# lucidrains/vector-quantize-pytorch

Measured on NVIDIA H100. Metric: vectors quantized/sec at dim=256, codebook=1024; indices bit-exact vs ref, higher is better.
Workload: dtype bf16

## Files before the change

### vector_quantize_pytorch_b200/csrc/epilogue.cuh

```cuda
#pragma once
#include <stdint.h>

namespace vqb {

__host__ __device__ __forceinline__ int group_col(int e) { return ((e >> 1) << 3) | (e & 1); }

__device__ __forceinline__ float fmax3(float a, float b, float c) { return fmaxf(fmaxf(a, b), c); }
template <int G>
__device__ __forceinline__ float max_group(const uint32_t* r) {
  static_assert(G == 4 || G == 8 || G == 16, "group size");
  if (G == 4) return fmaxf(fmax3(__uint_as_float(r[0]), __uint_as_float(r[1]), __uint_as_float(r[2])), __uint_as_float(r[3]));
  if (G == 8)
    return fmax3(fmax3(__uint_as_float(r[0]), __uint_as_float(r[1]), __uint_as_float(r[2])),
                 fmax3(__uint_as_float(r[3]), __uint_as_float(r[4]), __uint_as_float(r[5])),
                 fmaxf(__uint_as_float(r[6]), __uint_as_float(r[7])));
  const float a = fmax3(__uint_as_float(r[0]), __uint_as_float(r[1]), __uint_as_float(r[2]));
  const float b = fmax3(__uint_as_float(r[3]), __uint_as_float(r[4]), __uint_as_float(r[5]));
  const float c = fmax3(__uint_as_float(r[6]), __uint_as_float(r[7]), __uint_as_float(r[8]));
  const float d = fmax3(__uint_as_float(r[9]), __uint_as_float(r[10]), __uint_as_float(r[11]));
  const float e = fmax3(__uint_as_float(r[12]), __uint_as_float(r[13]), __uint_as_float(r[14]));
  return fmaxf(fmax3(a, b, c), fmax3(d, e, __uint_as_float(r[15])));
}
__device__ __forceinline__ float max16(const uint32_t (&r)[16]) { return max_group<16>(r); }

// ... 9 lines not shown
  template <int G>
  __device__ __forceinline__ void insert(const uint32_t* r, int cbase, uint32_t tagmask, uint32_t mul1, uint32_t mulm1) {
    const float o1 = t1, o2 = t2, o3 = t3;
#pragma unroll
    for (int e = 0; e < G; ++e) {
      const uint32_t ku = (r[e] & tagmask) | static_cast<uint32_t>(15 - e);
      const float n1 = fmaxf(t1, __uint_as_float(ku));
      const uint32_t lo1 = __float_as_uint(n1) * mulm1 + (__float_as_uint(t1) * mul1 + ku);
      const float n2 = fmaxf(t2, __uint_as_float(lo1));
      const uint32_t lo2 = __float_as_uint(n2) * mulm1 + (__float_as_uint(t2) * mul1 + lo1);
      const float n3 = fmaxf(t3, __uint_as_float(lo2));
      const uint32_t lo3 = __float_as_uint(n3) * mulm1 + (__float_as_uint(t3) * mul1 + lo2);
      t4 = fmaxf(t4, __uint_as_float(lo3));
      t1 = n1;
      t2 = n2;
      t3 = n3;
    }
    const int k1 = j1, k2 = j2, k3 = j3;
    const bool m1 = t1 == o1;
    j1 = m1 ? k1 : cbase;
    const float q2 = m1 ? o2 : o1;
    const bool m2 = t2 == q2;
    j2 = m2 ? (m1 ? k2 : k1) : cbase;
    const int used = static_cast<int>(m1) + static_cast<int>(m2);
    const float q3 = used == 0 ? o1 : (used == 1 ? o2 : o3);
    j3 = (t3 == q3) ? (used == 0 ? k1 : (used == 1 ? k2 : k3)) : cbase;
    thr = t1 - W;
  }
  __device__ __forceinline__ void piece(const uint32_t (&r)[16], int cbase, uint32_t tagmask, uint32_t mul1, uint32_t mulm1) {
    insert<16>(r, cbase, tagmask, mul1, mulm1);
  }
  static __device__ __forceinline__ int col(float t, int j) { return j + group_col(15 - static_cast<int>(__float_as_uint(t) & 15u)); }
};

struct MergeSlot { float t1, t2, t3, t4, bexact; int i0, i1, i2; };

struct RowResult { int i0, i1, i2, n; float best; };

struct Top3 {
  float v0 = -3.4e38f, v1 = -3.4e38f, v2 = -3.4e38f;
  int i0 = 0, i1 = 0, i2 = 0;
  __device__ __forceinline__ void offer(float v, int i) {
    if (v > v0 || (v == v0 && i < i0)) { v2 = v1; i2 = i1; v1 = v0; i1 = i0; v0 = v; i0 = i; }
    else if (v > v1 || (v == v1 && i < i1)) { v2 = v1; i2 = i1; v1 = v; i1 = i; }
    else if (v > v2 || (v == v2 && i < i2)) { v2 = v; i2 = i; }
  }
};

__device__ __forceinline__ void publish(MergeSlot* slot, const RowState& st) {
  slot->t1 = st.t1; slot->t2 = st.t2; slot->t3 = st.t3; slot->t4 = st.t4; slot->bexact = st.bexact;
  slot->i0 = RowState::col(st.t1, st.j1); slot->i1 = RowState::col(st.t2, st.j2); slot->i2 = RowState::col(st.t3, st.j3);
}

__device__ __forceinline__ RowResult merge_slices(const RowState& st, const MergeSlot* slots, int nslots, int stride) {
  float best = st.bexact, tb = st.t1;
  int ib = RowState::col(st.t1, st.j1);
  for (int q = 0; q < nslots; ++q) {
    const MergeSlot& m = slots[q * stride];
    best = fmaxf(best, m.bexact);
    const bool take = m.t1 > tb || (m.t1 == tb && m.i0 < ib);
    tb = take ? m.t1 : tb;
    ib = take ? m.i0 : ib;
  }
  const float band = tb - st.W;
  int n = (st.t1 > band) + (st.t2 > band) + (st.t3 > band) + (st.t4 > band);
  for (int q = 0; q < nslots; ++q) {
    const MergeSlot& m = slots[q * stride];
    n += (m.t1 > band) + (m.t2 > band) + (m.t3 > band) + (m.t4 > band);
  }
  RowResult r;
  r.i0 = ib; r.i1 = 0; r.i2 = 0; r.n = n; r.best = best;
  if (n >= 2) {
    Top3 top;
    top.offer(st.t1, RowState::col(st.t1, st.j1));
    top.offer(st.t2, RowState::col(st.t2, st.j2));
    top.offer(st.t3, RowState::col(st.t3, st.j3));
    for (int q = 0; q < nslots; ++q) {
      const MergeSlot& m = slots[q * stride];
      top.offer(m.t1, m.i0);
      top.offer(m.t2, m.i1);
      top.offer(m.t3, m.i2);
    }
    r.i0 = top.i0; r.i1 = top.i1; r.i2 = top.i2;
  }
  return r;
}

template <int G>
struct ScanQueue {
  static constexpr int CAP = 4;
  uint4 v[CAP + 1][G / 4];
  int c[CAP + 1];
};

template <int G>
struct ScanState {
  static constexpr int CAP = ScanQueue<G>::CAP;
  float t1;
  float thr;
  float kill;
  float W;
  int cnt;

  __device__ __forceinline__ void init(float w) {
    W = w; t1 = -3.4e38f; thr = -3.4e38f; kill = -3.4e38f; cnt = 0;
  }
  __device__ __forceinline__ void raise(float other) { thr = fmaxf(thr, other - W); }

  __device__ __forceinline__ void push(ScanQueue<G>& q, const uint32_t* r, int col, float m, bool p) {
    const int c0 = (m > kill) ? 0 : cnt;
    const int slot = min(c0, CAP);
    if (p) {
#pragma unroll
      for (int e = 0; e < G; e += 4) q.v[slot][e >> 2] = make_uint4(r[e], r[e + 1], r[e + 2], r[e + 3]);
      q.c[slot] = col;
    }
    cnt = p ? min(c0 + 1, CAP + 1) : cnt;
    t1 = fmaxf(t1, m);
    thr = fmaxf(thr, t1 - W);
    kill = t1 + W;
  }

  template <bool BRANCH = true>
  __device__ __forceinline__ void scan16(ScanQueue<G>& q, const uint32_t (&r)[16], int cbase) {
    float m[16 / G];
    bool any = false;
#pragma unroll
    for (int g = 0; g < 16 / G; ++g) {
      m[g] = max_group<G>(r + g * G);
// ... 112 lines not shown
```

### vector_quantize_pytorch_b200/csrc/ptx.cuh

```cuda
#pragma once
#include <cuda.h>
#include <cuda_runtime.h>
#include <stdint.h>

namespace vqb {

__device__ __forceinline__ uint32_t smem_u32(const void* p) {
  return static_cast<uint32_t>(__cvta_generic_to_shared(p));
}

__device__ __forceinline__ void mbar_init(uint32_t bar, uint32_t count) {
  asm volatile("mbarrier.init.shared::cta.b64 [%0], %1;" ::"r"(bar), "r"(count));
}
__device__ __forceinline__ void fence_barrier_init() {
  asm volatile("fence.mbarrier_init.release.cluster;" ::: "memory");
}
__device__ __forceinline__ void mbar_arrive(uint32_t bar) {
  asm volatile("mbarrier.arrive.shared::cta.b64 _, [%0];" ::"r"(bar) : "memory");
}
__device__ __forceinline__ void mbar_arrive_expect_tx(uint32_t bar, uint32_t bytes) {
  asm volatile("mbarrier.arrive.expect_tx.shared::cta.b64 _, [%0], %1;" ::"r"(bar), "r"(bytes) : "memory");
}
__device__ __forceinline__ bool mbar_try_wait(uint32_t bar, uint32_t parity) {
  uint32_t ok;
  asm volatile(
      "{\n"
      ".reg .pred p;\n"
      "mbarrier.try_wait.parity.shared::cta.b64 p, [%1], %2;\n"
      "selp.u32 %0, 1, 0, p;\n"
      "}\n"
      : "=r"(ok)
      : "r"(bar), "r"(parity)
      : "memory");
  return ok != 0;
}

#ifndef VQB_WAIT_TIMEOUT_CYCLES
#define VQB_WAIT_TIMEOUT_CYCLES (8000000000ll)
#endif
__device__ __forceinline__ void mbar_wait(uint32_t bar, uint32_t parity) {
  if (mbar_try_wait(bar, parity)) return;
  const long long t0 = clock64();
  while (!mbar_try_wait(bar, parity)) {
    if (clock64() - t0 > VQB_WAIT_TIMEOUT_CYCLES) __trap();
  }
}

__device__ __forceinline__ void tma_prefetch_desc(const CUtensorMap* m) {
  asm volatile("prefetch.tensormap [%0];" ::"l"(reinterpret_cast<uint64_t>(m)) : "memory");
}
__device__ __forceinline__ void tma_load_3d(uint32_t dst, const CUtensorMap* m, uint32_t bar, int c0, int c1, int c2) {
  asm volatile(
      "cp.async.bulk.tensor.3d.shared::cluster.global.tile.mbarrier::complete_tx::bytes [%0], [%1, {%3, %4, %5}], [%2];"
      ::"r"(dst), "l"(reinterpret_cast<uint64_t>(m)), "r"(bar), "r"(c0), "r"(c1), "r"(c2)
      : "memory");
}

__device__ __forceinline__ void tma_prefetch_l2_3d(const CUtensorMap* m, int c0, int c1, int c2) {
  asm volatile("cp.async.bulk.prefetch.tensor.3d.L2.global.tile [%0, {%1, %2, %3}];"
               ::"l"(reinterpret_cast<uint64_t>(m)), "r"(c0), "r"(c1), "r"(c2)
               : "memory");
}

__device__ __forceinline__ uint64_t wgmma_desc_sw128(uint32_t saddr) {
  uint64_t d = 0;
  d |= static_cast<uint64_t>((saddr >> 4) & 0x3FFF);
  d |= static_cast<uint64_t>(1) << 16;
  d |= static_cast<uint64_t>(1024 >> 4) << 32;
  d |= static_cast<uint64_t>(1) << 62;
  return d;
}

__device__ __forceinline__ uint64_t wgmma_desc_sw32(uint32_t saddr) {
  uint64_t d = 0;
  d |= static_cast<uint64_t>((saddr >> 4) & 0x3FFF);
  d |= static_cast<uint64_t>(1) << 16;
  d |= static_cast<uint64_t>(256 >> 4) << 32;
  d |= static_cast<uint64_t>(3) << 62;
  return d;
}

__device__ __forceinline__ void fence_proxy_async_shared() { asm volatile("fence.proxy.async.shared::cta;" ::: "memory"); }
__device__ __forceinline__ void wgmma_fence() { asm volatile("wgmma.fence.sync.aligned;" ::: "memory"); }
__device__ __forceinline__ void wgmma_commit() { asm volatile("wgmma.commit_group.sync.aligned;" ::: "memory"); }
template <int N>
__device__ __forceinline__ void wgmma_wait() { asm volatile("wgmma.wait_group.sync.aligned %0;" ::"n"(N) : "memory"); }

template <int R>
__device__ __forceinline__ void fence_regs(float (&d)[R]) {
#pragma unroll
  for (int i = 0; i < R; ++i) asm volatile("" : "+f"(d[i])::"memory");
}

__device__ __forceinline__ void wgmma_m64n128k16_bf16(float (&d)[64], uint64_t adesc, uint64_t bdesc) {
  asm volatile(
      "{\n"
      "wgmma.mma_async.sync.aligned.m64n128k16.f32.bf16.bf16 "
      "{%0, %1, %2, %3, %4, %5, %6, %7, %8, %9, %10, %11, %12, %13, %14, %15, "
// ... 147 lines not shown
```

### vector_quantize_pytorch_b200/csrc/vq_assign.cu

```cuda
#include <type_traits>
#include "ptx.cuh"
#include "vqb_common.cuh"
#include "gather_row.cuh"
#include "epilogue.cuh"

#ifdef VQB_PROFILE
#define PROF_CLOCK() clock64()
#else
#define PROF_CLOCK() 0ll
#endif

namespace vqb {

constexpr int BM = 128;
constexpr int WM = 64;
constexpr int BN_STAGE = 128;
constexpr int BK = 64;
constexpr int A_SUB_BYTES = BM * BK * 2;
constexpr int B_SUB_BYTES = BN_STAGE * BK * 2;
constexpr int MAX_A_SUB = 8;
constexpr int MAX_STAGES = 8;
constexpr int NUM_CONSUMER_WARPS = 8;
constexpr int NUM_STORE_WARPS = 3;
constexpr int NUM_THREADS = 128 + NUM_CONSUMER_WARPS * 32;
constexpr int SMEM_CTRL_BYTES = 14336;
constexpr int SMEM_LIMIT = 232448;
constexpr int SEED_BYTES = BN_STAGE * 32;

struct AssignParams {
  int64_t N;
  int D, K, Kpad;
  int n_a, n_passes;
  int KB;
  int n_stages;
  int n_seed;
  int stream_a;
  const uint16_t* a_global;
  const uint16_t* bext;
  int num_row_tiles, num_code_steps;
  float margin_rel;
  const float* cmax;
  int32_t* idx;
  int32_t* idx_prov;
  int32_t* hist;
  int hist_shift;
  vqb_flag_entry* flagged;
  int32_t* flag_count;
  float* dbg_best;
  const uint8_t* row_mask;
  long long* prof;
  FusedOut fo;
  int copy_mode;
  int resid_mode;
  int metric;
  const uint16_t* b_hi;
  const float* cnorm2;
  uint32_t tagmask, mul1, mulm1;
};

struct Ctrl {
  uint64_t a_full[MAX_A_SUB], a_empty[MAX_A_SUB];
  uint64_t b_full[MAX_STAGES], b_empty[MAX_STAGES];
  uint64_t g_full[2], g_empty[2];
  int gidx[2][BM];
  MergeSlot merge[BM][3];
  float x2[BM];
};
static_assert(sizeof(Ctrl) <= SMEM_CTRL_BYTES, "control block too large");

template <int GB>
__device__ __forceinline__ float tail_rows(const FusedOut& fo, const int64_t (&rows)[GB], const int (&ks)[GB], int D, int lane) {
  if (fo.dtype == VQB_DTYPE_BF16) return gather_rows<VQB_DTYPE_BF16, GB>(fo, rows, ks, D, lane);
  return gather_rows<VQB_DTYPE_F32, GB>(fo, rows, ks, D, lane);
}

__device__ __forceinline__ float sq_diff16(const uint4& xa, const uint4& ca, bool bf) {
  const uint32_t xw[4] = {xa.x, xa.y, xa.z, xa.w}, cw[4] = {ca.x, ca.y, ca.z, ca.w};
  float s = 0.f;
#pragma unroll
  for (int e = 0; e < 4; ++e) {
    if (bf) {
      const float d0 = __uint_as_float(xw[e] << 16) - __uint_as_float(cw[e] << 16);
      const float d1 = __uint_as_float(xw[e] & 0xFFFF0000u) - __uint_as_float(cw[e] & 0xFFFF0000u);
      s += bf16_round(d0 * d0);
      s += bf16_round(d1 * d1);
    } else {
      const float d = __uint_as_float(xw[e]) - __uint_as_float(cw[e]);
      s += d * d;
    }
  }
  return s;
}

template <int WN>
struct StepLocals {
  float loss_ = 0.f;
  __device__ __forceinline__ float& loss() { return loss_; }
};
template <>
struct StepLocals<256> {
  static __device__ __forceinline__ float& loss() {
    __shared__ float s[NUM_CONSUMER_WARPS * 32];
    return s[threadIdx.x - 128];
  }
  static __device__ __forceinline__ uint32_t* bias_ones() {
    __shared__ __align__(256) uint32_t o[WM * 16 / 2];
    return o;
  }
  __device__ __forceinline__ StepLocals() { loss() = 0.f; }
};
constexpr int WIDE_STATIC_SMEM = NUM_CONSUMER_WARPS * 32 * 4 + WM * 16 * 2;

template <int TAIL, int WN>
__global__ void __launch_bounds__(NUM_THREADS, 1)
vq_assign_kernel(const __grid_constant__ CUtensorMap tmA, const __grid_constant__ CUtensorMap tmB,
                 const __grid_constant__ CUtensorMap tmS, const AssignParams p) {
  static_assert(WN == 128 || WN == 256, "code step width");
  constexpr int SPAN = WN / BN_STAGE;
  constexpr uint32_t STEP_SEED_BYTES = SPAN * SEED_BYTES;
  extern __shared__ __align__(1024) uint8_t smem[];
  Ctrl* ctrl = reinterpret_cast<Ctrl*>(smem);
  const uint32_t smem_base = smem_u32(smem);
  const uint32_t a_base = (smem_base + SMEM_CTRL_BYTES + 1023u) & ~1023u;
  const bool stream_a = WN == 128 && p.stream_a;
  const int n_sub = stream_a ? 0 : p.n_a * p.KB;
  const uint32_t b_base = a_base + n_sub * A_SUB_BYTES;
  const uint32_t a_stage_bytes = stream_a ? A_SUB_BYTES : 0;
  const uint32_t stage_stride = a_stage_bytes + SPAN * B_SUB_BYTES;
  const int n_ring = p.n_stages / SPAN;
  const uint32_t seed_base = b_base + n_ring * stage_stride;

  const int warp = threadIdx.x >> 5;
  const int lane = threadIdx.x & 31;

  if (threadIdx.x == 0) {
    tma_prefetch_desc(&tmA);
    tma_prefetch_desc(&tmB);
    tma_prefetch_desc(&tmS);
    for (int s = 0; s < n_sub; ++s) {
      mbar_init(smem_u32(&ctrl->a_full[s]), 1);
      mbar_init(smem_u32(&ctrl->a_empty[s]), NUM_CONSUMER_WARPS);
    }
    for (int s = 0; s < n_ring; ++s) {
      mbar_init(smem_u32(&ctrl->b_full[s]), 1);
      mbar_init(smem_u32(&ctrl->b_empty[s]), NUM_CONSUMER_WARPS);
    }
    for (int s = 0; s < 2; ++s) {
      mbar_init(smem_u32(&ctrl->g_full[s]), NUM_CONSUMER_WARPS);
      mbar_init(smem_u32(&ctrl->g_empty[s]), NUM_STORE_WARPS);
    }
    fence_barrier_init();
  }
  if constexpr (WN == 256) {
    for (int i = threadIdx.x; i < WM * 16 / 2; i += NUM_THREADS) StepLocals<256>::bias_ones()[i] = 0x3F803F80u;
    fence_proxy_async_shared();
  }
  __syncthreads();

  if (warp == 0) {
    if (lane == 0) {
      long long w_empty = 0, w_aempty = 0;
      const long long pstart = PROF_CLOCK();
      int stage = 0, gstep = 0;
      uint32_t ph = 0;
      for (int t = 0, tile = static_cast<int>(blockIdx.x); tile < p.num_row_tiles; ++t, tile += static_cast<int>(gridDim.x)) {
        const int row0 = tile * BM;
        if (!stream_a && tile + static_cast<int>(gridDim.x) < p.num_row_tiles) {
          for (int ap = 0; ap < p.n_a; ++ap)
            for (int kb = 0; kb < p.KB; ++kb) tma_prefetch_l2_3d(&tmA, kb * BK, row0 + static_cast<int>(gridDim.x) * BM, ap);
        }
        for (int ct = 0; ct < p.num_code_steps; ++ct, ++gstep) {
          for (int kb = 0; kb < p.KB; ++kb) {
            for (int ps = 0; ps < p.n_passes; ++ps) {
              const int bplane = (ps == 1) ? 1 : 0;
              const int aplane = (ps == 2) ? 1 : 0;
              if (!stream_a && ct == 0 && (ps == 0 || ps == 2)) {
                const int sub = aplane * p.KB + kb;
                { const long long c0 = PROF_CLOCK(); mbar_wait(smem_u32(&ctrl->a_empty[sub]), (t & 1) ^ 1); w_aempty += PROF_CLOCK() - c0; }
                mbar_arrive_expect_tx(smem_u32(&ctrl->a_full[sub]), A_SUB_BYTES);
                tma_load_3d(a_base + sub * A_SUB_BYTES, &tmA, smem_u32(&ctrl->a_full[sub]), kb * BK, row0, aplane);
              }
              { const long long c0 = PROF_CLOCK(); mbar_wait(smem_u32(&ctrl->b_empty[stage]), ph ^ 1); w_empty += PROF_CLOCK() - c0; }
              const bool seeds = kb == 0 && ps == 0;
              mbar_arrive_expect_tx(smem_u32(&ctrl->b_full[stage]), stage_stride + (seeds ? STEP_SEED_BYTES : 0));
              if (seeds)
                tma_load_3d(seed_base + (gstep % p.n_seed) * STEP_SEED_BYTES, &tmS, smem_u32(&ctrl->b_full[stage]), 0, ct * WN, 0);
              if (stream_a)
                tma_load_3d(b_base + stage * stage_stride, &tmA, smem_u32(&ctrl->b_full[stage]), kb * BK, row0, aplane);
              tma_load_3d(b_base + stage * stage_stride + a_stage_bytes, &tmB, smem_u32(&ctrl->b_full[stage]), kb * BK,
                          ct * WN, bplane);
              if (++stage == n_ring) { stage = 0; ph ^= 1; }
            }
          }
        }
      }
      if (p.prof) {
        p.prof[blockIdx.x * 16 + 0] = w_empty;
        p.prof[blockIdx.x * 16 + 1] = PROF_CLOCK() - pstart;
        p.prof[blockIdx.x * 16 + 6] = w_aempty;
      }
    }
  } else if (warp <= NUM_STORE_WARPS) {
    const int sw = warp - 1;
    float lsum = 0.f;
    for (int t = 0, tile = static_cast<int>(blockIdx.x); p.fo.enabled && tile < p.num_row_tiles; ++t, tile += static_cast<int>(gridDim.x)) {
      mbar_wait(smem_u32(&ctrl->g_full[t & 1]), (t >> 1) & 1);
      const int* gi = ctrl->gidx[t & 1];
      if (TAIL >= 1) {
        constexpr int CB = 4;
        const bool bf = p.fo.dtype == VQB_DTYPE_BF16;
        const int row_bytes = p.D * (bf ? 2 : 4);
        const uint8_t* src = bf ? reinterpret_cast<const uint8_t*>(p.b_hi) : reinterpret_cast<const uint8_t*>(p.fo.embed);
        const uint8_t* xin = static_cast<const uint8_t*>(p.fo.x_eff);
        uint8_t* dst = static_cast<uint8_t*>(TAIL == 2 ? p.fo.resid_out : p.fo.q_out);
        for (int r0 = sw * CB; r0 < BM; r0 += NUM_STORE_WARPS * CB) {
          int ks[CB];
          bool ex[CB];
#pragma unroll
          for (int b = 0; b < CB; ++b) {
            const int g = gi[r0 + b];
            ex[b] = g < -1;
            ks[b] = ex[b] ? -2 - g : g;
          }
          const int64_t row_base = static_cast<int64_t>(tile) * BM + r0;
          if (p.fo.idx64_out && lane < CB && ks[lane & (CB - 1)] >= 0) {
            int kk = 0;
#pragma unroll
            for (int b = 0; b < CB; ++b) kk = (lane == b) ? ks[b] : kk;
            p.fo.idx64_out[(row_base + lane) * p.fo.idx_stride] = kk;
          }
          if (dst || (ex[0] | ex[1] | ex[2] | ex[3])) {
            for (int off = lane * 16; off < row_bytes; off += 512) {
              uint4 v[CB];
#pragma unroll
              for (int b = 0; b < CB; ++b)
                if (ks[b] >= 0) v[b] = __ldg(reinterpret_cast<const uint4*>(src + static_cast<int64_t>(ks[b]) * row_bytes + off));
              if (TAIL == 1) {
#pragma unroll
                for (int b = 0; b < CB; ++b)
                  if (ex[b]) lsum += sq_diff16(*reinterpret_cast<const uint4*>(xin + (row_base + b) * row_bytes + off), v[b], bf);
              }
              if (TAIL == 2) {
                uint4 x[CB];
#pragma unroll
                for (int b = 0; b < CB; ++b)
                  if (ks[b] >= 0) x[b] = *reinterpret_cast<const uint4*>(xin + (row_base + b) * row_bytes + off);
#pragma unroll
                for (int b = 0; b < CB; ++b) {
                  if (ks[b] < 0) continue;
                  if (ex[b]) lsum += sq_diff16(x[b], v[b], bf);
                  const uint32_t xw[4] = {x[b].x, x[b].y, x[b].z, x[b].w}, cw[4] = {v[b].x, v[b].y, v[b].z, v[b].w};
                  uint32_t rw[4];
                  if (bf) {
#pragma unroll
                    for (int e = 0; e < 4; ++e) {
                      const float d0 = __uint_as_float(xw[e] << 16) - __uint_as_float(cw[e] << 16);
                      const float d1 = __uint_as_float(xw[e] & 0xFFFF0000u) - __uint_as_float(cw[e] & 0xFFFF0000u);
                      asm("cvt.rn.bf16x2.f32 %0, %1, %2;" : "=r"(rw[e]) : "f"(d1), "f"(d0));
                    }
                  } else {
#pragma unroll
                    for (int e = 0; e < 4; ++e) rw[e] = __float_as_uint(__uint_as_float(xw[e]) - __uint_as_float(cw[e]));
                    if (p.fo.planes_out) {
                      const float rf[4] = {__uint_as_float(rw[0]), __uint_as_float(rw[1]), __uint_as_float(rw[2]), __uint_as_float(rw[3])};
                      store_planes4(p.fo.planes_out, p.fo.planes_stride, ((row_base + b) * row_bytes + off) >> 2, rf);
                    }
                  }
                  v[b] = make_uint4(rw[0], rw[1], rw[2], rw[3]);
                }
              }
#pragma unroll
              for (int b = 0; b < CB; ++b)
                if (dst && ks[b] >= 0) *reinterpret_cast<uint4*>(dst + (row_base + b) * row_bytes + off) = v[b];
            }
          }
        }
      } else {
        constexpr int GB = 2;
        for (int r0 = sw * GB; r0 < BM; r0 += NUM_STORE_WARPS * GB) {
          int64_t rows[GB];
          int ks[GB];
          bool any = false;
#pragma unroll
          for (int b = 0; b < GB; ++b) {
            ks[b] = gi[r0 + b];
            rows[b] = ks[b] >= 0 ? static_cast<int64_t>(tile) * BM + r0 + b : -1;
            any |= ks[b] >= 0;
          }
          if (!any) continue;
          lsum += tail_rows<GB>(p.fo, rows, ks, p.D, lane);
        }
      }
      __syncwarp();
      if (lane == 0) mbar_arrive(smem_u32(&ctrl->g_empty[t & 1]));
    }
    if (p.fo.enabled && p.fo.loss_sum) {
      const double w = warp_sum(static_cast<double>(lsum));
      if (lane == 0) atomicAdd(p.fo.loss_sum, w);
    }
  } else {
    const int wg = (warp >> 2) - 1;
    const int q = lane & 3;
    const int rit0 = wg * WM + (warp & 3) * 16 + (lane >> 2);
    const int n_items = p.KB * p.n_passes;
    const uint32_t a_row_off = wg * WM * 128;
    const uint32_t bias_a = q == 0 ? 0x3F803F80u : (q == 1 ? 0x00003F80u : 0u);
    long long w_full = 0, w_afull = 0, w_gap = 0, gap0 = -1;
    const long long cstart = PROF_CLOCK();
    float acc[WN / 2];
    int stage = 0, gstep = 0;
    uint32_t ph = 0;
    StepLocals<WN> locals;
    auto release = [&](int st, int sub) {
      if (lane == 0) {
        mbar_arrive(smem_u32(&ctrl->b_empty[st]));
        if (sub >= 0) mbar_arrive(smem_u32(&ctrl->a_empty[sub]));
      }
    };
    auto row_norms = [&](int tile, float (&xlo)[2]) {
#pragma unroll
      for (int h = 0; h < 2; ++h) {
        const int64_t row = static_cast<int64_t>(tile) * BM + rit0 + 8 * h;
        float a = 0.f, alo = 0.f;
        if (row < p.N) {
          const uint16_t* hp = p.a_global + row * p.D;
          for (int c = q * 8; c < p.D; c += 32) {
            const uint4 u = __ldg(reinterpret_cast<const uint4*>(hp + c));
            uint4 l = make_uint4(0u, 0u, 0u, 0u);
            if (p.n_a == 2) l = __ldg(reinterpret_cast<const uint4*>(hp + p.N * p.D + c));
            const uint32_t w[4] = {u.x, u.y, u.z, u.w};
            const uint32_t wl[4] = {l.x, l.y, l.z, l.w};
#pragma unroll
            for (int e = 0; e < 4; ++e) {
              const float h0 = __uint_as_float(w[e] << 16), h1 = __uint_as_float(w[e] & 0xFFFF0000u);
              const float l0 = __uint_as_float(wl[e] << 16), l1 = __uint_as_float(wl[e] & 0xFFFF0000u);
              a = fmaf(h0 + l0, h0 + l0, a);
              a = fmaf(h1 + l1, h1 + l1, a);
              alo = fmaf(l0, l0, alo);
              alo = fmaf(l1, l1, alo);
            }
          }
        }
        a += __shfl_xor_sync(0xffffffffu, a, 1);
        a += __shfl_xor_sync(0xffffffffu, a, 2);
        alo += __shfl_xor_sync(0xffffffffu, alo, 1);
        alo += __shfl_xor_sync(0xffffffffu, alo, 2);
        if (q == 0) ctrl->x2[rit0 + 8 * h] = a;
        xlo[h] = alo;
      }
    };
    auto init_band = [&](auto (&sc)[2], float (&xlo)[2]) {
      const bool euclid = p.metric != VQB_METRIC_COSINE;
      const float cmax = __ldg(p.cmax + CMAX_NORM);
      const float cres = __ldg(p.cmax + CMAX_RES);
      const float caux = p.n_a == 2 ? 0x1.02p-8f * cmax + __ldg(p.cmax + CMAX_LO) : 0.f;
      __syncwarp();
#pragma unroll
      for (int h = 0; h < 2; ++h) {
        const float x2 = ctrl->x2[rit0 + 8 * h];
        const float xn = sqrtf(x2);
        const float xc = xn * cmax;
        xlo[h] = p.n_a == 2 ? sqrtf(xlo[h]) * 1.0001f : 0.f;
        sc[h].init(2.f * (xn * cres + xlo[h] * caux + p.margin_rel * xc + (euclid ? 0x1p-21f * cmax * cmax : 0.f)) +
                   0x1p-18f * (xc + (euclid ? 0.5f * cmax * cmax : 0.f)) +
                   (euclid ? 0x1p-22f * (x2 + cmax * cmax) + 1e-8f : 1e-30f));
      }
    };
    for (int t = 0, tile = static_cast<int>(blockIdx.x); tile < p.num_row_tiles; ++t, tile += static_cast<int>(gridDim.x)) {
      typename std::conditional<WN == 128, ScanReg, ScanState<16>>::type sc[2];
      ScanQueue<16> sq[2];

      float xlo[2] = {0.f, 0.f};
      for (int ct = 0; ct < p.num_code_steps; ++ct) {
        const bool last_ct = ct == p.num_code_steps - 1;
        if (WN == 256 && ct == 0) {
          row_norms(tile, xlo);
          init_band(sc, xlo);
        }
        if (gap0 >= 0) w_gap += PROF_CLOCK() - gap0;
        { const long long c0 = PROF_CLOCK(); mbar_wait(smem_u32(&ctrl->b_full[stage]), ph); w_full += PROF_CLOCK() - c0; }
        wgmma_fence();
        const uint64_t sd = wgmma_desc_sw32(seed_base + (gstep % p.n_seed) * STEP_SEED_BYTES);
        if constexpr (WN == 128) wgmma_m64n128k16_bf16_rs_set(acc, bias_a, sd);
        else wgmma_m64n256k16_bf16_ss_set(acc, wgmma_desc_sw32(smem_u32(StepLocals<256>::bias_ones())), sd);
        int kb = 0, ps = 0;
        int pend_stage = -1, pend_sub = -1;
        for (int i = 0; i < n_items; ++i) {
          const int aplane = (ps == 2) ? 1 : 0;
          const int sub = aplane * p.KB + kb;
          if (ct == 0 && !stream_a) { const long long c0 = PROF_CLOCK(); mbar_wait(smem_u32(&ctrl->a_full[sub]), t & 1); w_afull += PROF_CLOCK() - c0; }
          if (i > 0) { const long long c0 = PROF_CLOCK(); mbar_wait(smem_u32(&ctrl->b_full[stage]), ph); w_full += PROF_CLOCK() - c0; }
          const uint32_t st_addr = b_base + stage * stage_stride;
          const uint32_t a_addr = (stream_a ? st_addr : a_base + sub * A_SUB_BYTES) + a_row_off;
          const uint64_t ad = wgmma_desc_sw128(a_addr);
          const uint64_t bd = wgmma_desc_sw128(st_addr + a_stage_bytes);
          fence_regs(acc);
          wgmma_fence();
#pragma unroll
          for (int k = 0; k < 8; k += 2) {
            if constexpr (WN == 128) wgmma_m64n128k16_bf16(acc, ad + k, bd + k);
            else wgmma_m64n256k16_bf16(acc, ad + k, bd + k);
          }
          wgmma_commit();
          if (i == n_items - 1) gap0 = PROF_CLOCK();
          wgmma_wait<1>();
          fence_regs(acc);
          if (pend_stage >= 0) release(pend_stage, pend_sub);
          const bool last_use = last_ct && !stream_a && (aplane == 1 ? ps == 2 : ps == 1);
          pend_stage = stage;
          pend_sub = last_use ? sub : -1;
          if (++stage == n_ring) { stage = 0; ph ^= 1; }
          if (++ps == p.n_passes) { ps = 0; ++kb; }
        }
        if (WN == 128 && ct == 0) row_norms(tile, xlo);
        wgmma_wait<0>();
        fence_regs(acc);
        release(pend_stage, pend_sub);
        ++gstep;
        if ((ct + 1) * WN > p.Kpad) {
#pragma unroll
          for (int j = 0; j < WN / 8; ++j)
#pragma unroll
            for (int b = 0; b < 2; ++b)
              if (ct * WN + 8 * j + 2 * q + b >= p.Kpad) { acc[4 * j + b] = -3.0e38f; acc[4 * j + 2 + b] = -3.0e38f; }
        }

        if (WN == 128 && ct == 0) {
          init_band(sc, xlo);
        } else if (ct > 0) {
#pragma unroll
          for (int h = 0; h < 2; ++h) {
            float m = sc[h].t1;
            m = fmaxf(m, __shfl_xor_sync(0xffffffffu, m, 1));
            m = fmaxf(m, __shfl_xor_sync(0xffffffffu, m, 2));
            sc[h].raise(m);
          }
        }
#pragma unroll
        for (int g = 0; g < WN / 64; ++g) {
#pragma unroll
          for (int h = 0; h < 2; ++h) {
            uint32_t r[16];
#pragma unroll
            for (int e = 0; e < 16; ++e) r[e] = __float_as_uint(acc[4 * (8 * g + (e >> 1)) + 2 * h + (e & 1)]);
            if constexpr (WN == 128) sc[h].template scan16<true, false>(sq[h], r, ct * WN + 64 * g + 2 * q, p.mul1);
            else sc[h].template scan16<true>(sq[h], r, ct * WN + 64 * g + 2 * q);
          }
        }
      }

      if (p.fo.enabled) mbar_wait(smem_u32(&ctrl->g_empty[t & 1]), ((t >> 1) & 1) ^ 1);
#pragma unroll
      for (int h = 0; h < 2; ++h) {
        const int rit = rit0 + 8 * h;
        RowState st;
        sc[h].finish(sq[h], st, p.tagmask, p.mul1, p.mulm1);
        MergeSlot* slots = ctrl->merge[rit];
        if (q != 0) publish(&slots[q - 1], st);
        __syncwarp();
        if (q == 0) {
          const RowResult rr = merge_slices(st, slots, 3, 1);
          const int n = rr.n, i0 = rr.i0, i1 = rr.i1;
          const float best = rr.best;
          const int64_t row = static_cast<int64_t>(tile) * BM + rit;
          const bool live = row < p.N && (p.row_mask == nullptr || __ldg(p.row_mask + row) != 0);
          bool exact_loss = false;
          if (TAIL >= 1 && p.fo.loss_sum && live && n < 2) {
            float d2 = ctrl->x2[rit] - 2.f * best;
            if (p.metric == VQB_METRIC_COSINE) d2 += __ldg(p.cnorm2 + i0);
            exact_loss = !(d2 >= 0x1p14f * st.W);
            if (!exact_loss) locals.loss() += d2;
          }
          if (p.fo.enabled) ctrl->gidx[t & 1][rit] = (live && n < 2) ? (exact_loss ? -2 - i0 : i0) : -1;
          if (row < p.N && !live) {
            p.idx[row] = -1;
            if (p.idx_prov) p.idx_prov[row] = -1;
          } else if (row < p.N) {
            p.idx[row] = i0;
            if (p.idx_prov) p.idx_prov[row] = (n < 2) ? i0 : -1;
            if (p.hist && n < 2) atomicAdd(p.hist + static_cast<size_t>(tile >> p.hist_shift) * p.K + i0, 1);
            if (p.dbg_best) p.dbg_best[row] = best;
            if (n >= 2) {
              const bool many = n > 3;
              const int s = many ? static_cast<int>(p.N) - 1 - atomicAdd(p.flag_count + 1, 1) : atomicAdd(p.flag_count, 1);
              vqb_flag_entry e;
              e.row = static_cast<int32_t>(row);
              e.cand0 = many ? 0 : i0;
              e.cand1 = many ? 0 : i1;
              e.cand2 = rr.i2;
              e.count = n;
              e.pad[0] = e.pad[1] = e.pad[2] = 0;
              p.flagged[s] = e;
            }
          }
        }
        __syncwarp();
      }
      if (p.fo.enabled && lane == 0) mbar_arrive(smem_u32(&ctrl->g_full[t & 1]));
    }
    if (TAIL >= 1 && p.fo.loss_sum) {
      const double w = warp_sum(static_cast<double>(locals.loss()));
      if (lane == 0) atomicAdd(p.fo.loss_sum, w);
    }
    if (p.prof && threadIdx.x == 128) {
      p.prof[blockIdx.x * 16 + 2] = w_full;
      p.prof[blockIdx.x * 16 + 3] = PROF_CLOCK() - cstart;
      p.prof[blockIdx.x * 16 + 4] = w_gap;
      p.prof[blockIdx.x * 16 + 5] = w_afull;
    }
  }
}

typedef CUresult (*PFN_encodeTiled)(CUtensorMap*, CUtensorMapDataType, cuuint32_t, void*, const cuuint64_t*,
                                    const cuuint64_t*, const cuuint32_t*, const cuuint32_t*, CUtensorMapInterleave,
                                    CUtensorMapSwizzle, CUtensorMapL2promotion, CUtensorMapFloatOOBfill);

static PFN_encodeTiled get_encode_fn() {
  static PFN_encodeTiled fn = nullptr;
  static bool tried = false;
  if (!tried) {
    tried = true;
    void* f = nullptr;
    cudaDriverEntryPointQueryResult qres;
    if (cudaGetDriverEntryPoint("cuTensorMapEncodeTiled", &f, cudaEnableDefault, &qres) == cudaSuccess &&
        qres == cudaDriverEntryPointSuccess)
      fn = reinterpret_cast<PFN_encodeTiled>(f);
  }
  return fn;
}

static int make_map(CUtensorMap* m, const void* base, int cols, int64_t rows, int planes, int box_cols, int box_rows,
                    CUtensorMapSwizzle swz) {
  PFN_encodeTiled enc = get_encode_fn();
  if (!enc) return VQB_E_DRIVER;
  cuuint64_t dims[3] = {static_cast<cuuint64_t>(cols), static_cast<cuuint64_t>(rows), static_cast<cuuint64_t>(planes)};
  cuuint64_t strides[2] = {static_cast<cuuint64_t>(cols) * 2, static_cast<cuuint64_t>(cols) * 2 * static_cast<cuuint64_t>(rows)};
  cuuint32_t box[3] = {static_cast<cuuint32_t>(box_cols), static_cast<cuuint32_t>(box_rows), 1};
  cuuint32_t estr[3] = {1, 1, 1};
  CUresult r = enc(m, CU_TENSOR_MAP_DATA_TYPE_BFLOAT16, 3, const_cast<void*>(base), dims, strides, box, estr,
                   CU_TENSOR_MAP_INTERLEAVE_NONE, swz, CU_TENSOR_MAP_L2_PROMOTION_L2_256B, CU_TENSOR_MAP_FLOAT_OOB_FILL_NONE);
  return r == CUDA_SUCCESS ? VQB_OK : VQB_E_DRIVER;
}

struct AssignPlan {
  int stream_a, n_stages, n_seed, n_items, KB, smem_bytes;
};

static int assign_plan(int n_a, int D, int n_passes, AssignPlan* pl) {
  if (D <= 0 || (n_a != 1 && n_a != 2)) return VQB_E_INVALID;
  if (n_passes == 0) n_passes = n_a + 1;
  if (n_passes != n_a + 1) return VQB_E_UNSUPPORTED;
  if (D % 8 != 0) return VQB_E_UNSUPPORTED;
  const int KB = (D + BK - 1) / BK;
  const int stream_a = n_a * KB > MAX_A_SUB ? 1 : 0;
  const int a_bytes = stream_a ? 0 : n_a * KB * A_SUB_BYTES;
  const int stage_bytes = B_SUB_BYTES + (stream_a ? A_SUB_BYTES : 0);
  const int fixed = SMEM_CTRL_BYTES + 1024  + a_bytes;
  const int n_items = KB * n_passes;
  int stages = MAX_STAGES;
  auto seed_slots = [&](int st) { return (st + n_items - 1) / n_items; };
  while (stages >= 2 && fixed + stages * stage_bytes + seed_slots(stages) * SEED_BYTES > SMEM_LIMIT) --stages;
// ... 141 lines not shown
```

Baseline: 391.1 million.

## Offload row norms and cross-slice merge to store warps in wide path

```diff
diff --git a/vector_quantize_pytorch_b200/csrc/epilogue.cuh b/vector_quantize_pytorch_b200/csrc/epilogue.cuh
--- a/vector_quantize_pytorch_b200/csrc/epilogue.cuh
+++ b/vector_quantize_pytorch_b200/csrc/epilogue.cuh
@@ -85,9 +85,9 @@
   slot->i0 = RowState::col(st.t1, st.j1); slot->i1 = RowState::col(st.t2, st.j2); slot->i2 = RowState::col(st.t3, st.j3);
 }
 
-__device__ __forceinline__ RowResult merge_slices(const RowState& st, const MergeSlot* slots, int nslots, int stride) {
-  float best = st.bexact, tb = st.t1;
-  int ib = RowState::col(st.t1, st.j1);
+__device__ __forceinline__ RowResult merge_slices(const MergeSlot& own, float W, const MergeSlot* slots, int nslots, int stride) {
+  float best = own.bexact, tb = own.t1;
+  int ib = own.i0;
   for (int q = 0; q < nslots; ++q) {
     const MergeSlot& m = slots[q * stride];
     best = fmaxf(best, m.bexact);
@@ -95,8 +95,8 @@
     tb = take ? m.t1 : tb;
     ib = take ? m.i0 : ib;
   }
-  const float band = tb - st.W;
-  int n = (st.t1 > band) + (st.t2 > band) + (st.t3 > band) + (st.t4 > band);
+  const float band = tb - W;
+  int n = (own.t1 > band) + (own.t2 > band) + (own.t3 > band) + (own.t4 > band);
   for (int q = 0; q < nslots; ++q) {
     const MergeSlot& m = slots[q * stride];
     n += (m.t1 > band) + (m.t2 > band) + (m.t3 > band) + (m.t4 > band);
@@ -105,9 +105,9 @@
   r.i0 = ib; r.i1 = 0; r.i2 = 0; r.n = n; r.best = best;
   if (n >= 2) {
     Top3 top;
-    top.offer(st.t1, RowState::col(st.t1, st.j1));
-    top.offer(st.t2, RowState::col(st.t2, st.j2));
-    top.offer(st.t3, RowState::col(st.t3, st.j3));
+    top.offer(own.t1, own.i0);
+    top.offer(own.t2, own.i1);
+    top.offer(own.t3, own.i2);
     for (int q = 0; q < nslots; ++q) {
       const MergeSlot& m = slots[q * stride];
       top.offer(m.t1, m.i0);
diff --git a/vector_quantize_pytorch_b200/csrc/ptx.cuh b/vector_quantize_pytorch_b200/csrc/ptx.cuh
--- a/vector_quantize_pytorch_b200/csrc/ptx.cuh
+++ b/vector_quantize_pytorch_b200/csrc/ptx.cuh
@@ -44,6 +44,10 @@
   while (!mbar_try_wait(bar, parity)) {
     if (clock64() - t0 > VQB_WAIT_TIMEOUT_CYCLES) __trap();
   }
+}
+
+__device__ __forceinline__ void named_bar_sync(uint32_t id, uint32_t count) {
+  asm volatile("bar.sync %0, %1;" ::"r"(id), "r"(count) : "memory");
 }
 
 __device__ __forceinline__ void tma_prefetch_desc(const CUtensorMap* m) {
diff --git a/vector_quantize_pytorch_b200/csrc/vq_assign.cu b/vector_quantize_pytorch_b200/csrc/vq_assign.cu
--- a/vector_quantize_pytorch_b200/csrc/vq_assign.cu
+++ b/vector_quantize_pytorch_b200/csrc/vq_assign.cu
@@ -62,6 +62,8 @@
   uint64_t a_full[MAX_A_SUB], a_empty[MAX_A_SUB];
   uint64_t b_full[MAX_STAGES], b_empty[MAX_STAGES];
   uint64_t g_full[2], g_empty[2];
+  uint64_t norm_full[2], norm_empty[2];
+  uint64_t merge_full, merge_empty;
   int gidx[2][BM];
   MergeSlot merge[BM][3];
   float x2[BM];
@@ -92,24 +94,142 @@
   return s;
 }
 
+template <int R>
+__device__ __forceinline__ void row_norms2(const AssignParams& p, const int (&row)[R], int q, float (&x2)[R],
+                                           float (&xlo2)[R]) {
+  float a[R], alo[R];
+#pragma unroll
+  for (int j = 0; j < R; ++j) a[j] = alo[j] = 0.f;
+  if (p.n_a == 1) {
+    for (int c = q * 8; c < p.D; c += 32) {
+      uint4 u[R];
+#pragma unroll
+      for (int j = 0; j < R; ++j)
+        u[j] = row[j] < p.N ? __ldg(reinterpret_cast<const uint4*>(p.a_global + static_cast<int64_t>(row[j]) * p.D + c))
+                            : make_uint4(0u, 0u, 0u, 0u);
+#pragma unroll
+      for (int j = 0; j < R; ++j) {
+        const uint32_t w[4] = {u[j].x, u[j].y, u[j].z, u[j].w};
+#pragma unroll
+        for (int e = 0; e < 4; ++e) {
+          const float h0 = __uint_as_float(w[e] << 16), h1 = __uint_as_float(w[e] & 0xFFFF0000u);
+          a[j] = fmaf(h0, h0, a[j]);
+          a[j] = fmaf(h1, h1, a[j]);
+        }
+      }
+    }
+  } else {
+    for (int c = q * 8; c < p.D; c += 32) {
+      uint4 u[R], l[R];
+#pragma unroll
+      for (int j = 0; j < R; ++j) {
+        u[j] = l[j] = make_uint4(0u, 0u, 0u, 0u);
+        if (row[j] < p.N) {
+          const uint16_t* hp = p.a_global + static_cast<int64_t>(row[j]) * p.D;
+          u[j] = __ldg(reinterpret_cast<const uint4*>(hp + c));
+          l[j] = __ldg(reinterpret_cast<const uint4*>(hp + p.N * p.D + c));
+        }
+      }
+#pragma unroll
+      for (int j = 0; j < R; ++j) {
+        const uint32_t w[4] = {u[j].x, u[j].y, u[j].z, u[j].w};
+        const uint32_t wl[4] = {l[j].x, l[j].y, l[j].z, l[j].w};
+#pragma unroll
+        for (int e = 0; e < 4; ++e) {
+          const float h0 = __uint_as_float(w[e] << 16), h1 = __uint_as_float(w[e] & 0xFFFF0000u);
+          const float l0 = __uint_as_float(wl[e] << 16), l1 = __uint_as_float(wl[e] & 0xFFFF0000u);
+          a[j] = fmaf(h0 + l0, h0 + l0, a[j]);
+          a[j] = fmaf(h1 + l1, h1 + l1, a[j]);
+          alo[j] = fmaf(l0, l0, alo[j]);
+          alo[j] = fmaf(l1, l1, alo[j]);
+        }
+      }
+    }
+  }
+#pragma unroll
+  for (int j = 0; j < R; ++j) {
+    a[j] += __shfl_xor_sync(0xffffffffu, a[j], 1);
+    a[j] += __shfl_xor_sync(0xffffffffu, a[j], 2);
+    alo[j] += __shfl_xor_sync(0xffffffffu, alo[j], 1);
+    alo[j] += __shfl_xor_sync(0xffffffffu, alo[j], 2);
+    x2[j] = a[j];
+    xlo2[j] = alo[j];
+  }
+}
+
+__device__ __forceinline__ float row_band(const AssignParams& p, float x2, float xlo2) {
+  const bool euclid = p.metric != VQB_METRIC_COSINE;
+  const float cmax = __ldg(p.cmax + CMAX_NORM);
+  const float cres = __ldg(p.cmax + CMAX_RES);
+  const float caux = p.n_a == 2 ? 0x1.02p-8f * cmax + __ldg(p.cmax + CMAX_LO) : 0.f;
+  const float xn = sqrtf(x2);
+  const float xc = xn * cmax;
+  const float xlo = p.n_a == 2 ? sqrtf(xlo2) * 1.0001f : 0.f;
+  return 2.f * (xn * cres + xlo * caux + p.margin_rel * xc + (euclid ? 0x1p-21f * cmax * cmax : 0.f)) +
+         0x1p-18f * (xc + (euclid ? 0.5f * cmax * cmax : 0.f)) +
+         (euclid ? 0x1p-22f * (x2 + cmax * cmax) + 1e-8f : 1e-30f);
+}
+
+template <int TAIL>
+__device__ __forceinline__ int row_outputs(const AssignParams& p, const RowResult& rr, int tile, int rit, float x2, float W,
+                                           float& loss) {
+  const int n = rr.n, i0 = rr.i0, i1 = rr.i1;
+  const float best = rr.best;
+  const int64_t row = static_cast<int64_t>(tile) * BM + rit;
+  const bool live = row < p.N && (p.row_mask == nullptr || __ldg(p.row_mask + row) != 0);
+  bool exact_loss = false;
+  if (TAIL >= 1 && p.fo.loss_sum && live && n < 2) {
+    float d2 = x2 - 2.f * best;
+    if (p.metric == VQB_METRIC_COSINE) d2 += __ldg(p.cnorm2 + i0);
+    exact_loss = !(d2 >= 0x1p14f * W);
+    if (!exact_loss) loss += d2;
+  }
+  if (row < p.N && !live) {
+    p.idx[row] = -1;
+    if (p.idx_prov) p.idx_prov[row] = -1;
+  } else if (row < p.N) {
+    p.idx[row] = i0;
+    if (p.idx_prov) p.idx_prov[row] = (n < 2) ? i0 : -1;
+    if (p.hist && n < 2) atomicAdd(p.hist + static_cast<size_t>(tile >> p.hist_shift) * p.K + i0, 1);
+    if (p.dbg_best) p.dbg_best[row] = best;
+    if (n >= 2) {
+      const bool many = n > 3;
+      const int s = many ? static_cast<int>(p.N) - 1 - atomicAdd(p.flag_count + 1, 1) : atomicAdd(p.flag_count, 1);
+      vqb_flag_entry e;
+      e.row = static_cast<int32_t>(row);
+      e.cand0 = many ? 0 : i0;
+      e.cand1 = many ? 0 : i1;
+      e.cand2 = rr.i2;
+      e.count = n;
+      e.pad[0] = e.pad[1] = e.pad[2] = 0;
+      p.flagged[s] = e;
+    }
+  }
+  return (live && n < 2) ? (exact_loss ? -2 - i0 : i0) : -1;
+}
+
 template <int WN>
 struct StepLocals {
   float loss_ = 0.f;
   __device__ __forceinline__ float& loss() { return loss_; }
 };
+struct TileNorms { float x2[BM], W[BM]; };
 template <>
 struct StepLocals<256> {
-  static __device__ __forceinline__ float& loss() {
-    __shared__ float s[NUM_CONSUMER_WARPS * 32];
-    return s[threadIdx.x - 128];
-  }
   static __device__ __forceinline__ uint32_t* bias_ones() {
     __shared__ __align__(256) uint32_t o[WM * 16 / 2];
     return o;
   }
-  __device__ __forceinline__ StepLocals() { loss() = 0.f; }
+  static __device__ __forceinline__ MergeSlot* slot0() {
+    __shared__ MergeSlot s[BM];
+    return s;
+  }
+  static __device__ __forceinline__ TileNorms* norms() {
+    __shared__ TileNorms n[2];
+    return n;
+  }
 };
-constexpr int WIDE_STATIC_SMEM = NUM_CONSUMER_WARPS * 32 * 4 + WM * 16 * 2;
+constexpr int WIDE_STATIC_SMEM = WM * 16 * 2 + BM * static_cast<int>(sizeof(MergeSlot)) + 2 * static_cast<int>(sizeof(TileNorms));
 
 template <int TAIL, int WN>
 __global__ void __launch_bounds__(NUM_THREADS, 1)
@@ -146,8 +266,17 @@
       mbar_init(smem_u32(&ctrl->b_empty[s]), NUM_CONSUMER_WARPS);
     }
     for (int s = 0; s < 2; ++s) {
-      mbar_init(smem_u32(&ctrl->g_full[s]), NUM_CONSUMER_WARPS);
-      mbar_init(smem_u32(&ctrl->g_empty[s]), NUM_STORE_WARPS);
+      if constexpr (WN == 128) {
+        mbar_init(smem_u32(&ctrl->g_full[s]), NUM_CONSUMER_WARPS);
+        mbar_init(smem_u32(&ctrl->g_empty[s]), NUM_STORE_WARPS);
+      } else {
+        mbar_init(smem_u32(&ctrl->norm_full[s]), NUM_STORE_WARPS);
+        mbar_init(smem_u32(&ctrl->norm_empty[s]), NUM_CONSUMER_WARPS);
+      }
+    }
+    if constexpr (WN == 256) {
+      mbar_init(smem_u32(&ctrl->merge_full), NUM_CONSUMER_WARPS);
+      mbar_init(smem_u32(&ctrl->merge_empty), 1);
     }
     fence_barrier_init();
   }
@@ -203,9 +332,9 @@
   } else if (warp <= NUM_STORE_WARPS) {
     const int sw = warp - 1;
     float lsum = 0.f;
-    for (int t = 0, tile = static_cast<int>(blockIdx.x); p.fo.enabled && tile < p.num_row_tiles; ++t, tile += static_cast<int>(gridDim.x)) {
-      mbar_wait(smem_u32(&ctrl->g_full[t & 1]), (t >> 1) & 1);
-      const int* gi = ctrl->gidx[t & 1];
+    long long w_busy = 0;
+    long long w_norms = 0, w_merge = 0;
+    auto tail = [&](int tile, const int* gi) {
       if (TAIL >= 1) {
         constexpr int CB = 4;
         const bool bf = p.fo.dtype == VQB_DTYPE_BF16;
@@ -291,8 +420,67 @@
           lsum += tail_rows<GB>(p.fo, rows, ks, p.D, lane);
         }
       }
-      __syncwarp();
-      if (lane == 0) mbar_arrive(smem_u32(&ctrl->g_empty[t & 1]));
+    };
+    if constexpr (WN == 256) {
+      auto tile_norms = [&](int t, int tile) {
+        mbar_wait(smem_u32(&ctrl->norm_empty[t & 1]), ((t >> 1) & 1) ^ 1);
+        const long long b0 = PROF_CLOCK();
+        TileNorms& nb = StepLocals<256>::norms()[t & 1];
+        constexpr int RW = (BM + NUM_STORE_WARPS * 8 - 1) / (NUM_STORE_WARPS * 8);
+        int rows[RW];
+        float x2[RW], xlo2[RW];
+#pragma unroll
+        for (int i = 0; i < RW; ++i) {
+          const int r = sw * 8 + (lane >> 2) + NUM_STORE_WARPS * 8 * i;
+          rows[i] = r < BM ? tile * BM + r : static_cast<int>(p.N);
+        }
+        row_norms2<RW>(p, rows, lane & 3, x2, xlo2);
+        if ((lane & 3) == 0) {
+#pragma unroll
+          for (int i = 0; i < RW; ++i) {
+            const int r = sw * 8 + (lane >> 2) + NUM_STORE_WARPS * 8 * i;
+            if (r < BM) {
+              nb.x2[r] = x2[i];
+              nb.W[r] = row_band(p, x2[i], xlo2[i]);
+            }
+          }
+        }
+        __syncwarp();
+        if (lane == 0) mbar_arrive(smem_u32(&ctrl->norm_full[t & 1]));
+        w_busy += PROF_CLOCK() - b0;
+        w_norms += PROF_CLOCK() - b0;
+      };
+      tile_norms(0, static_cast<int>(blockIdx.x));
+      for (int t = 0, tile = static_cast<int>(blockIdx.x); tile < p.num_row_tiles; ++t, tile += static_cast<int>(gridDim.x)) {
+        if (tile + static_cast<int>(gridDim.x) < p.num_row_tiles) tile_norms(t + 1, tile + static_cast<int>(gridDim.x));
+        mbar_wait(smem_u32(&ctrl->merge_full), t & 1);
+        const long long b0 = PROF_CLOCK();
+        const TileNorms& nb = StepLocals<256>::norms()[t & 1];
+        int* gi = ctrl->gidx[t & 1];
+        for (int r = threadIdx.x - 32; r < BM; r += NUM_STORE_WARPS * 32) {
+          const RowResult rr = merge_slices(StepLocals<256>::slot0()[r], nb.W[r], ctrl->merge[r], 3, 1);
+          gi[r] = row_outputs<TAIL>(p, rr, tile, r, nb.x2[r], nb.W[r], lsum);
+        }
+        named_bar_sync(1, NUM_STORE_WARPS * 32);
+        if (threadIdx.x == 32) mbar_arrive(smem_u32(&ctrl->merge_empty));
+        w_merge += PROF_CLOCK() - b0;
+        if (p.fo.enabled) tail(tile, gi);
+        w_busy += PROF_CLOCK() - b0;
+      }
+    } else {
+      for (int t = 0, tile = static_cast<int>(blockIdx.x); p.fo.enabled && tile < p.num_row_tiles; ++t, tile += static_cast<int>(gridDim.x)) {
+        mbar_wait(smem_u32(&ctrl->g_full[t & 1]), (t >> 1) & 1);
+        const long long b0 = PROF_CLOCK();
+        tail(tile, ctrl->gidx[t & 1]);
+        __syncwarp();
+        w_busy += PROF_CLOCK() - b0;
+        if (lane == 0) mbar_arrive(smem_u32(&ctrl->g_empty[t & 1]));
+      }
+    }
+    if (p.prof && threadIdx.x == 32) {
+      p.prof[blockIdx.x * 16 + 8] = w_busy;
+      p.prof[blockIdx.x * 16 + 9] = w_norms;
+      p.prof[blockIdx.x * 16 + 10] = w_merge;
     }
     if (p.fo.enabled && p.fo.loss_sum) {
       const double w = warp_sum(static_cast<double>(lsum));
@@ -306,6 +494,7 @@
     const uint32_t a_row_off = wg * WM * 128;
     const uint32_t bias_a = q == 0 ? 0x3F803F80u : (q == 1 ? 0x00003F80u : 0u);
     long long w_full = 0, w_afull = 0, w_gap = 0, gap0 = -1;
+    long long w_bound = 0;
     const long long cstart = PROF_CLOCK();
     float acc[WN / 2];
     int stage = 0, gstep = 0;
@@ -320,65 +509,31 @@
     auto row_norms = [&](int tile, float (&xlo)[2]) {
 #pragma unroll
       for (int h = 0; h < 2; ++h) {
-        const int64_t row = static_cast<int64_t>(tile) * BM + rit0 + 8 * h;
-        float a = 0.f, alo = 0.f;
-        if (row < p.N) {
-          const uint16_t* hp = p.a_global + row * p.D;
-          for (int c = q * 8; c < p.D; c += 32) {
-            const uint4 u = __ldg(reinterpret_cast<const uint4*>(hp + c));
-            uint4 l = make_uint4(0u, 0u, 0u, 0u);
-            if (p.n_a == 2) l = __ldg(reinterpret_cast<const uint4*>(hp + p.N * p.D + c));
-            const uint32_t w[4] = {u.x, u.y, u.z, u.w};
-            const uint32_t wl[4] = {l.x, l.y, l.z, l.w};
-#pragma unroll
-            for (int e = 0; e < 4; ++e) {
-              const float h0 = __uint_as_float(w[e] << 16), h1 = __uint_as_float(w[e] & 0xFFFF0000u);
-              const float l0 = __uint_as_float(wl[e] << 16), l1 = __uint_as_float(wl[e] & 0xFFFF0000u);
-              a = fmaf(h0 + l0, h0 + l0, a);
-              a = fmaf(h1 + l1, h1 + l1, a);
-              alo = fmaf(l0, l0, alo);
-              alo = fmaf(l1, l1, alo);
-            }
-          }
-        }
-        a += __shfl_xor_sync(0xffffffffu, a, 1);
-        a += __shfl_xor_sync(0xffffffffu, a, 2);
-        alo += __shfl_xor_sync(0xffffffffu, alo, 1);
-        alo += __shfl_xor_sync(0xffffffffu, alo, 2);
-        if (q == 0) ctrl->x2[rit0 + 8 * h] = a;
-        xlo[h] = alo;
+        const int row[1] = {tile * BM + rit0 + 8 * h};
+        float a[1], alo[1];
+        row_norms2<1>(p, row, q, a, alo);
+        if (q == 0) ctrl->x2[rit0 + 8 * h] = a[0];
+        xlo[h] = alo[0];
       }
     };
     auto init_band = [&](auto (&sc)[2], float (&xlo)[2]) {
-      const bool euclid = p.metric != VQB_METRIC_COSINE;
-      const float cmax = __ldg(p.cmax + CMAX_NORM);
-      const float cres = __ldg(p.cmax + CMAX_RES);
-      const float caux = p.n_a == 2 ? 0x1.02p-8f * cmax + __ldg(p.cmax + CMAX_LO) : 0.f;
       __syncwarp();
 #pragma unroll
-      for (int h = 0; h < 2; ++h) {
-        const float x2 = ctrl->x2[rit0 + 8 * h];
-        const float xn = sqrtf(x2);
-        const float xc = xn * cmax;
-        xlo[h] = p.n_a == 2 ? sqrtf(xlo[h]) * 1.0001f : 0.f;
-        sc[h].init(2.f * (xn * cres + xlo[h] * caux + p.margin_rel * xc + (euclid ? 0x1p-21f * cmax * cmax : 0.f)) +
-                   0x1p-18f * (xc + (euclid ? 0.5f * cmax * cmax : 0.f)) +
-                   (euclid ? 0x1p-22f * (x2 + cmax * cmax) + 1e-8f : 1e-30f));
-      }
+      for (int h = 0; h < 2; ++h) sc[h].init(row_band(p, ctrl->x2[rit0 + 8 * h], xlo[h]));
     };
-    for (int t = 0, tile = static_cast<int>(blockIdx.x); tile < p.num_row_tiles; ++t, tile += static_cast<int>(gridDim.x)) {
+    for (int t = 0; static_cast<int>(blockIdx.x + t * gridDim.x) < p.num_row_tiles; ++t) {
+      const int tile = static_cast<int>(blockIdx.x + t * gridDim.x);
       typename std::conditional<WN == 128, ScanReg, ScanState<16>>::type sc[2];
       ScanQueue<16> sq[2];
 
       float xlo[2] = {0.f, 0.f};
       for (int ct = 0; ct < p.num_code_steps; ++ct) {
         const bool last_ct = ct == p.num_code_steps - 1;
-        if (WN == 256 && ct == 0) {
-          row_norms(tile, xlo);
-          init_band(sc, xlo);
-        }
         if (gap0 >= 0) w_gap += PROF_CLOCK() - gap0;
         { const long long c0 = PROF_CLOCK(); mbar_wait(smem_u32(&ctrl->b_full[stage]), ph); w_full += PROF_CLOCK() - c0; }
+#ifdef VQB_PROFILE
+        if (ct == 0 && gap0 >= 0) w_bound += PROF_CLOCK() - gap0;
+#endif
         wgmma_fence();
         const uint64_t sd = wgmma_desc_sw32(seed_base + (gstep % p.n_seed) * STEP_SEED_BYTES);
         if constexpr (WN == 128) wgmma_m64n128k16_bf16_rs_set(acc, bias_a, sd);
@@ -425,9 +580,18 @@
               if (ct * WN + 8 * j + 2 * q + b >= p.Kpad) { acc[4 * j + b] = -3.0e38f; acc[4 * j + 2 + b] = -3.0e38f; }
         }
 
-        if (WN == 128 && ct == 0) {
-          init_band(sc, xlo);
-        } else if (ct > 0) {
+        if (ct == 0) {
+          if constexpr (WN == 128) {
+            init_band(sc, xlo);
+          } else {
+            mbar_wait(smem_u32(&ctrl->norm_full[t & 1]), (t >> 1) & 1);
+            const float* W = StepLocals<256>::norms()[t & 1].W;
+#pragma unroll
+            for (int h = 0; h < 2; ++h) sc[h].init(W[rit0 + 8 * h]);
+            __syncwarp();
+            if (lane == 0) mbar_arrive(smem_u32(&ctrl->norm_empty[t & 1]));
+          }
+        } else {
 #pragma unroll
           for (int h = 0; h < 2; ++h) {
             float m = sc[h].t1;
@@ -449,64 +613,51 @@
         }
       }
 
-      if (p.fo.enabled) mbar_wait(smem_u32(&ctrl->g_empty[t & 1]), ((t >> 1) & 1) ^ 1);
-#pragma unroll
-      for (int h = 0; h < 2; ++h) {
-        const int rit = rit0 + 8 * h;
-        RowState st;
-        sc[h].finish(sq[h], st, p.tagmask, p.mul1, p.mulm1);
-        MergeSlot* slots = ctrl->merge[rit];
-        if (q != 0) publish(&slots[q - 1], st);
+      if constexpr (WN == 256) {
+        mbar_wait(smem_u32(&ctrl->merge_empty), (t & 1) ^ 1);
+#pragma unroll
+        for (int h = 0; h < 2; ++h) {
+          const int rit = rit0 + 8 * h;
+          RowState st;
+          sc[h].finish(sq[h], st, p.tagmask, p.mul1, p.mulm1);
+          publish(q == 0 ? &StepLocals<256>::slot0()[rit] : &ctrl->merge[rit][q - 1], st);
+        }
         __syncwarp();
-        if (q == 0) {
-          const RowResult rr = merge_slices(st, slots, 3, 1);
-          const int n = rr.n, i0 = rr.i0, i1 = rr.i1;
-          const float best = rr.best;
-          const int64_t row = static_cast<int64_t>(tile) * BM + rit;
-          const bool live = row < p.N && (p.row_mask == nullptr || __ldg(p.row_mask + row) != 0);
-          bool exact_loss = false;
-          if (TAIL >= 1 && p.fo.loss_sum && live && n < 2) {
-            float d2 = ctrl->x2[rit] - 2.f * best;
-            if (p.metric == VQB_METRIC_COSINE) d2 += __ldg(p.cnorm2 + i0);
-            exact_loss = !(d2 >= 0x1p14f * st.W);
-            if (!exact_loss) locals.loss() += d2;
-          }
-          if (p.fo.enabled) ctrl->gidx[t & 1][rit] = (live && n < 2) ? (exact_loss ? -2 - i0 : i0) : -1;
-          if (row < p.N && !live) {
-            p.idx[row] = -1;
-            if (p.idx_prov) p.idx_prov[row] = -1;
-          } else if (row < p.N) {
-            p.idx[row] = i0;
-            if (p.idx_prov) p.idx_prov[row] = (n < 2) ? i0 : -1;
-            if (p.hist && n < 2) atomicAdd(p.hist + static_cast<size_t>(tile >> p.hist_shift) * p.K + i0, 1);
-            if (p.dbg_best) p.dbg_best[row] = best;
-            if (n >= 2) {
-              const bool many = n > 3;
-              const int s = many ? static_cast<int>(p.N) - 1 - atomicAdd(p.flag_count + 1, 1) : atomicAdd(p.flag_count, 1);
-              vqb_flag_entry e;
-              e.row = static_cast<int32_t>(row);
-              e.cand0 = many ? 0 : i0;
-              e.cand1 = many ? 0 : i1;
-              e.cand2 = rr.i2;
-              e.count = n;
-              e.pad[0] = e.pad[1] = e.pad[2] = 0;
-              p.flagged[s] = e;
-            }
-          }
-        }
-        __syncwarp();
-      }
-      if (p.fo.enabled && lane == 0) mbar_arrive(smem_u32(&ctrl->g_full[t & 1]));
-    }
-    if (TAIL >= 1 && p.fo.loss_sum) {
-      const double w = warp_sum(static_cast<double>(locals.loss()));
-      if (lane == 0) atomicAdd(p.fo.loss_sum, w);
+        if (lane == 0) mbar_arrive(smem_u32(&ctrl->merge_full));
+      } else {
+        if (p.fo.enabled) mbar_wait(smem_u32(&ctrl->g_empty[t & 1]), ((t >> 1) & 1) ^ 1);
+#pragma unroll
+        for (int h = 0; h < 2; ++h) {
+          const int rit = rit0 + 8 * h;
+          RowState st;
+          sc[h].finish(sq[h], st, p.tagmask, p.mul1, p.mulm1);
+          MergeSlot* slots = ctrl->merge[rit];
+          if (q != 0) publish(&slots[q - 1], st);
+          __syncwarp();
+          if (q == 0) {
+            MergeSlot own;
+            publish(&own, st);
+            const RowResult rr = merge_slices(own, st.W, slots, 3, 1);
+            const int g = row_outputs<TAIL>(p, rr, tile, rit, ctrl->x2[rit], st.W, locals.loss());
+            if (p.fo.enabled) ctrl->gidx[t & 1][rit] = g;
+          }
+          __syncwarp();
+        }
+        if (p.fo.enabled && lane == 0) mbar_arrive(smem_u32(&ctrl->g_full[t & 1]));
+      }
+    }
+    if constexpr (WN == 128) {
+      if (TAIL >= 1 && p.fo.loss_sum) {
+        const double w = warp_sum(static_cast<double>(locals.loss()));
+        if (lane == 0) atomicAdd(p.fo.loss_sum, w);
+      }
     }
     if (p.prof && threadIdx.x == 128) {
       p.prof[blockIdx.x * 16 + 2] = w_full;
       p.prof[blockIdx.x * 16 + 3] = PROF_CLOCK() - cstart;
       p.prof[blockIdx.x * 16 + 4] = w_gap;
       p.prof[blockIdx.x * 16 + 5] = w_afull;
+      p.prof[blockIdx.x * 16 + 7] = w_bound;
     }
   }
 }
```

New measurement: 410.0 million, median of 6. +4.8%, better.
